# fvalka/atc-reinforcement-learning

Measured on AMD Instinct MI355X. Metric: env-steps/sec aggregate @16 aircraft/env, 64k envs, higher is better.
Workload: dtype f32

## Files before the change

### atc-reinforcement-learning_amd/csrc/atc_step.hip

```cpp
#include <hip/hip_runtime.h>
#include <atomic>
#include <chrono>
#include <sched.h>
#include <emmintrin.h>
#include <stdint.h>
#include <stdio.h>
#include <string.h>

#include "atc_device.h"

using namespace atc;

struct atc_scenario {
    float* d_blob;
    int n_words;
    int off_grid;
    int device;
    int n_cu;
    float consts[ATC_C_END];
    float ghdr[ATC_G_HDR];
    uint64_t uid;
    void* d_lds;
    LdsTab lt;
    size_t lds_tab_bytes;
// ... 641 lines not shown
            const float t2 = in_horizon ? lim.sep2 : lim.sep2_h, tf = in_horizon ? lim.sep_ft : lim.sep_ft_h;
#pragma unroll 1
            for (int d0 = H - U + 1; d0 >= 1; d0 -= U) {
                const int batch = (d0 - 1) / U;
                if (kHZ && !((batches >> batch) & 1u)) continue;
                v2f qx[U / 2], qy[U / 2], qh[U / 2];
#pragma unroll
                for (int u = 0; u < U / 2; ++u) {
                    const float* q0 = own + d0 + 2 * u;
                    qx[u] = v2f{q0[0], q0[1]};
                    qy[u] = v2f{q0[P], q0[P + 1]};
                    qh[u] = v2f{q0[2 * P], q0[2 * P + 1]};
                }
                uint64_t mk[U];
                v2f d2k[U / 2], dhk[U / 2];
#pragma unroll
                for (int u = U / 2 - 1; u >= 0; --u) {
                    const v2f dx = xs2 - qx[u], dy = ys2 - qy[u];
                    const v2f d2 = __builtin_elementwise_fma(dx, dx, dy * dy);
                    d2k[u] = d2;
                    {
                        const v2f dh = hs2 - qh[u];
                        dhk[u] = dh;
                        mk[2 * u] = __builtin_amdgcn_ballot_w64(d2[0] < t2) & __builtin_amdgcn_ballot_w64(fabsf(dh[0]) < tf);
                        mk[2 * u + 1] = __builtin_amdgcn_ballot_w64(d2[1] < t2) & __builtin_amdgcn_ballot_w64(fabsf(dh[1]) < tf);
                    }
                    if (FULL) {
#pragma unroll
                        for (int w = 1; w >= 0; --w) {
                            const int dd = d0 + 2 * u + w;
                            min_d2 = fminf(min_d2, d2[w]);
                            atomicMin(reinterpret_cast<unsigned int*>(own - k + 3 * P + ((k + dd) & (W - 1))), __float_as_uint(d2[w]));
                        }
                    }
                }
                uint64_t any = mk[0];
#pragma unroll
                for (int j = 1; j < U; ++j) any |= mk[j];
                if (ATC_RARE(any != 0ull)) {
                    if (kHZ && !in_horizon) {
                        flagged |= 1u << batch;
                        any = 0ull;
#pragma unroll
                        for (int j = 0; j < U; ++j) {
                            mk[j] = __builtin_amdgcn_ballot_w64(d2k[j / 2][j % 2] < sep2) & __builtin_amdgcn_ballot_w64(fabsf(dhk[j / 2][j % 2]) < sep_ft);
                            any |= mk[j];
                        }
                    }
                    hit |= any;
#pragma unroll
                    for (int j = 0; j < U; ++j) {
                        const int dd = d0 + j;
                        const uint64_t t = mk[j];
                        if (W == 64) {
                            hit |= (t << dd) | (t >> (64 - dd));
                        } else {
                            const uint32_t lo = (uint32_t)t, hi = (uint32_t)(t >> 32);
                            hit |= (uint64_t)((lo << dd) | (lo >> (32 - dd))) | ((uint64_t)((hi << dd) | (hi >> (32 - dd))) << 32);
                        }
                    }
                }
            }
            if ((hit >> lane) & 1ull) margin = -1.0f;
            if (FULL) {
                __builtin_amdgcn_fence(__ATOMIC_RELEASE, "wavefront");
                __builtin_amdgcn_wave_barrier();
                __builtin_amdgcn_fence(__ATOMIC_ACQUIRE, "wavefront");
                min_d2 = fminf(min_d2, own[3 * P]);
            }
            __builtin_amdgcn_wave_barrier();
        }
        if (kHZ && !in_horizon) {
            const uint64_t odd = __builtin_amdgcn_ballot_w64(a.v > kVMaxFix) | __builtin_amdgcn_ballot_w64(!(fabsf(hf) < kScanHMax));
            scan_skip = (odd != 0ull) ? 0 : kHorizon;
            scan_mask = flagged;
        }
    }
    ATC_STAMP_B(2);
    Obs ob;
    float shaping = 0.0f;
    const ObsConst oc = QGET(oc);
    constexpr bool kPrefetch = (W == 1 || (ONE && W == 16)) && kResolveAfterScan && !LDSG;
    constexpr bool kObsFirst = kPrefetch || W == 1;
    MvaPre pre;
    if (kPrefetch) pre = mva_prefetch(grid, QGET(g.gh), m.cell);
    if (kObsFirst) {
        const WideWords wo = LAT ? ww : wide_words<ONE>(m.plain, a.phi, wide_named, zk, i);
        const float phi_f = phi_real(wo.counts), phi_o = __int_as_float(wo.obs_bits);
        ob = get_state(oc, a.x, a.y, x32, y32, hf, phi_f, phi_o, v_real(a.v), hf);
        if (p.mode & ATC_M_REWARD_SHAPING) shaping = shaping_total(shaping_core(oc, ob.d_faf, ob.phi_rel_faf, ob.o[9], hf, ob.on_gp));
    }
    ATC_STAMP_TOP(so.trace, 5);
    if (LDSG) {
        float hgt = 0.0f;
        uint32_t walk;
        bool band;
        pi = lds_resolve(ltab, *lt, m.lc, x32, y32, &hgt, &walk, &band);
        if (ATC_RARE(__builtin_amdgcn_ballot_w64(walk != 0u) != 0ull)) {
            if (walk != 0u) pi = lds_walk(*lt, walk, x32, y32, &hgt);
            asm volatile("" : "+v"(pi), "+v"(hgt));
        }
        if (ATC_RARE(__builtin_amdgcn_ballot_w64(band) != 0ull)) {
            const GridHdr gh = QGET(g.gh);
            const MvaCell c = mva_cell_load(grid, gh, x32, y32);
            pi = mva_resolve<kWalkBatch>(K, grid, gh, c, x32, y32, &hgt);
            asm volatile("" : "+v"(pi), "+v"(hgt));
        }
        mva = hgt;
    } else if (kResolveAfterScan) {
        float hgt = 0.0f;
        pi = mva_resolve<kWalkBatch>(K, grid, QGET(g.gh), m.cell, x32, y32, &hgt, kPrefetch ? &pre : nullptr);
        mva = hgt;
        fl |= noise_areas(K, grid, qs.n_noise, m.cell, x32, y32, a.h);
    }
    ATC_STAMP_END(so.trace, 1);
    const bool conflict = margin < 0.0f;
    const bool timeout = es.t > qs.timestep_limit;
    const uint64_t in_tri = LDSG ? __builtin_amdgcn_ballot_w64(lds_corridor_candidate(m.lc))
                          : grid ? __builtin_amdgcn_ballot_w64(corridor_candidate(m.cell))
                                 : (__builtin_amdgcn_ballot_w64(x32 >= qs.tri_bbox.x) & __builtin_amdgcn_ballot_w64(x32 <= qs.tri_bbox.z) &
                                    __builtin_amdgcn_ballot_w64(y32 >= qs.tri_bbox.y) & __builtin_amdgcn_ballot_w64(y32 <= qs.tri_bbox.w));
    const double mva_d = (double)mva;
    const bool quiet = m.plain &&
                       (__builtin_amdgcn_ballot_w64(pi < 0) | __builtin_amdgcn_ballot_w64(a.h < mva_d) | __builtin_amdgcn_ballot_w64(margin < 0.0f) |
                        __builtin_amdgcn_ballot_w64(es.t > qs.timestep_limit) | __builtin_amdgcn_ballot_w64(fl > 0xffffu) | in_tri) == 0ull;
    if (ATC_RARE(!quiet)) {
        {
            const bool below = pi >= 0 && a.h < mva_d;
            r = pi < 0 ? -50.0f : (below ? -200.0f : r);
            fl |= pi < 0 ? (uint32_t)ATC_F_OUTSIDE : (below ? (uint32_t)ATC_F_BELOW_MVA : 0u);
        }
        {
            r = conflict ? qs.conflict_reward : r;
            fl |= conflict ? (uint32_t)ATC_F_CONFLICT : 0u;
        }
        if (inside_corridor(K, qs.tri_bbox, x32, y32, hf, (double)(LAT ? ww.counts : heading_counts<ONE>(m.plain, a.phi, wide_named, zk, i)))) {
            int bonus = (qs.timestep_limit - es.t) * 5;
            bonus = bonus < 0 ? 0 : bonus;
            r = (float)(10000 + bonus);
            fl |= ATC_F_WON;
        }
        {
            r = timeout ? -200.0f : r;
            fl |= timeout ? (uint32_t)ATC_F_TIMEOUT : 0u;
        }
    }
    ATC_STAMP_B(3);
    ATC_STAMP_END(so.trace, 2);
    const QNorm qn = QGET(n);
    float o[ATC_OBS_DIM];
    float zraw[ATC_OBS_DIM];
    {
        if (kObsFirst) {
            ob.o[5] = alt_above(a.h, mva);
        } else {
            const WideWords wo = LAT ? ww : wide_words<ONE>(m.plain, a.phi, wide_named, zk, i);
            const float phi_f = phi_real(wo.counts), phi_o = __int_as_float(wo.obs_bits);
            ob = get_state(oc, a.x, a.y, x32, y32, hf, phi_f, phi_o, v_real(a.v), alt_above(a.h, mva));
            if (p.mode & ATC_M_REWARD_SHAPING) shaping = shaping_total(shaping_core(oc, ob.d_faf, ob.phi_rel_faf, ob.o[9], hf, ob.on_gp));
        }
        if (p.mode & ATC_M_REWARD_SHAPING) r += shaping;
        if (ATC_RARE(!quiet && __builtin_amdgcn_ballot_w64((fl >> 16) != 0u) != 0ull)) {
            const int n_noise = qs.n_noise;
            for (int q = 0; q < n_noise; ++q)
                if ((fl >> (16 + q)) & 1u) r -= (K + (int)K[ATC_H_OFF_POLY] + ((int)K[ATC_H_N_MVA] + q) * ATC_P_WORDS)[ATC_P_PENALTY];
            fl &= 0xffffu;
        }
        if (FULL) {
#pragma unroll
            for (int c = 0; c < ATC_OBS_DIM; ++c) zraw[c] = active ? ob.o[c] : 0.0f;
            if (so.raw_obs && d.lane_valid) store_obs(at<float>(so.raw_obs, times40(i)), zraw);
        }
#pragma unroll
        for (int c = 0; c < ATC_OBS_DIM; ++c) o[c] = fmaf(ob.o[c], qn.a[c], qn.b[c]);
    }
    if (ATC_RARE(!m.plain && __builtin_amdgcn_ballot_w64(!active) != 0ull)) {
#pragma unroll
        for (int c = 0; c < ATC_OBS_DIM; ++c) o[c] = active ? o[c] : 0.0f;
        r = active ? r : 0.0f;
        acts = active ? acts : 0;
        fl = active ? fl : (d.lane_valid ? (uint32_t)ATC_F_INACTIVE : 0u);
        if (!active) min_d2 = 1e30f;
    }

    ATC_STAMP_B(4);
    ATC_STAMP_END(so.trace, 3);
    const float env_r = group_sum<W>(r);
    const int env_acts = m.repeated ? 0 : group_sum_i<W>(acts);
    bool done = false, env_won = false;
    if (ATC_RARE(!quiet)) {
        const uint64_t won = group_ballot<W>((fl & ATC_F_WON) != 0, lane);
        const uint64_t term = group_ballot<W>(
            (fl & (ATC_F_BELOW_MVA | ATC_F_OUTSIDE | ATC_F_CONFLICT | ATC_F_TIMEOUT)) != 0, lane);
        const bool keep_active = (p.mode & ATC_M_KEEP_ACTIVE) != 0;
        if (!keep_active) es.amask &= ~won;
        env_won = keep_active ? won != 0 : es.amask == 0;
        done = d.env_valid && (term != 0 || env_won);
        if (kHZ && (p.mode & ATC_M_AUTO_RESET) && __builtin_amdgcn_ballot_w64(done) != 0ull) scan_skip = 0;
    }
    es.total_reward += env_r;
    es.n_actions += env_acts;

    if (FULL && ONE && W == 1 && so.packet && d.lane_valid) {
        const uint32_t tag = p.reserved0;
        const float w[27] = {o[0], o[1], o[2], o[3], o[4], o[5], o[6], o[7], o[8], o[9], zraw[0], zraw[1], zraw[2], zraw[3],
                             zraw[4], zraw[5], zraw[6], zraw[7], zraw[8], zraw[9], env_r,
                             __uint_as_float((fl & 0xffffu) | (done ? 0x10000u : 0u)), __int_as_float(es.t),
                             __int_as_float(es.n_actions), __int_as_float(a.x), __int_as_float(a.y), 0.0f};
        uint4* pk = at<uint4>(so.packet, (uint32_t)e * (ATC_PKT_CHUNKS * 16u));
#pragma unroll
        for (int c = 0; c < ATC_PKT_CHUNKS; ++c)
            store16_system(pk + c, __float_as_uint(w[3 * c]), __float_as_uint(w[3 * c + 1]), __float_as_uint(w[3 * c + 2]), tag);
    }
    if (FULL && so.min_sep) {
        const float m2 = (W > 1) ? group_min<W>(min_d2) : 1e30f;
        if (d.env_valid && k == 0) *at<float>(so.min_sep, (uint32_t)e * 4u) = (m2 >= 1e30f) ? 1e30f : sqrtf(m2);
    }

    if (ATC_RARE(done && (p.mode & ATC_M_AUTO_RESET))) {
        __builtin_amdgcn_fence(__ATOMIC_ACQUIRE, "wavefront");
        int32_t* stats = ONE ? stp : kernarg_reread<int32_t*>(offsetof(StepArgs, st) + offsetof(atc_state_t, stats), zk);
        int4* sr = at<int4>(stats, (uint32_t)e * (ATC_STAT_WORDS * 4u));
        const int4 s0 = sr[0];
        const int episode = s0.x;
        if (d.env_valid && k == 0) {
            const uint32_t win_bits = (((uint32_t)s0.w << 1) | (env_won ? 1u : 0u)) & 0x3ffu;
            sr[0] = make_int4(episode + 1, es.t, __float_as_int(es.total_reward), (int)win_bits);
            *at<int>(stats, (uint32_t)e * (ATC_STAT_WORDS * 4u) + ATC_STAT_EP_ACTIONS * 4u) = es.n_actions;
        }
        __builtin_amdgcn_fence(__ATOMIC_RELEASE, "wavefront");
        if (d.lane_valid) {
            if (FULL && so.term_obs) store_obs(at<float>(so.term_obs, times40(i)), o);
            a = spawn(K, qs.off_spawn, p, e, k + zk, episode, o);
        }
        es.total_reward = 0.0f;
        es.n_actions = 0;
        es.t = 0;
        es.amask = (N >= 64) ? ~0ull : ((1ull << N) - 1ull);
    }

    ATC_STAMP_B(5);
    ATC_STAMP_END(so.trace, 4);
    if (!ONE && !LAT) {
        int zn;
        asm volatile("s_mov_b32 %0, 0" : "=s"(zn));
        qr_next = kernarg_reread<QRates>(offsetof(StepArgs, q) + offsetof(StepDerived, r), zn);
    }
    if (ATC_RARE(act_next != nullptr)) asm volatile("" : "+v"(a_next.a), "+v"(a_next.b), "+v"(a_next.c));
    if (ATC_USUAL(d.wave_full)) {
        const uint32_t ln = threadIdx.x & 63u, wv = threadIdx.x >> 6;
        float* tb = obs_stage + __umul24(wv, 64u * ATC_OBS_DIM);
        float2* tb2 = reinterpret_cast<float2*>(tb) + __umul24(ln, ATC_OBS_DIM / 2);
#pragma unroll
        for (int c = 0; c < ATC_OBS_DIM / 2; ++c) tb2[c] = make_float2(o[2 * c], o[2 * c + 1]);
        __builtin_amdgcn_fence(__ATOMIC_RELEASE, "wavefront");
        __builtin_amdgcn_wave_barrier();
        __builtin_amdgcn_fence(__ATOMIC_ACQUIRE, "wavefront");
        const uint32_t wave_off = (d.slot0 + (uint32_t)__builtin_amdgcn_readfirstlane((int)(threadIdx.x & ~63u))) * 40u;
        const float4* src = reinterpret_cast<const float4*>(tb);
#pragma unroll
        for (int j = 0; j < 3; ++j) {
            const uint32_t idx = (uint32_t)j * 64u + ln;
            if (idx < 64u * ATC_OBS_DIM / 4u) {
                const float4 v = src[idx];
                float* d4 = at<float>(so.obs, wave_off + idx * 16u);
                typedef float v4f __attribute__((ext_vector_type(4)));
                __builtin_nontemporal_store(v4f{v.x, v.y, v.z, v.w}, reinterpret_cast<v4f*>(d4));
            }
        }
        __builtin_amdgcn_wave_barrier();
    } else if (d.lane_valid) {
        store_obs(at<float>(so.obs, times40(i)), o);
    }
    ATC_STAMP_END(so.trace, 5);
    if (d.lane_valid) {
        stream_store(at<uint16_t>(so.flags, i * 2u), (uint16_t)fl);
        if (FULL && so.ac_reward) *at<float>(so.ac_reward, i * 4u) = r;
    }
    if (d.env_valid && k == 0) {
        *at<float>(so.reward, (uint32_t)e * 4u) = env_r;
        *at<uint8_t>(so.done, (uint32_t)e) = done ? 1 : 0;
    }
    return quiet;
}

__device__ __forceinline__ void store_lane_state(const atc_state_t& st, const LaneIds& d, const LaneState& ls, bool la_live) {
    if (d.lane_valid) {
        *at<int4>(st.ac, d.i * 16u) = make_int4(ls.a.x, ls.a.y, ls.a.phi, (int)ls.a.v);
        *at<double>(st.alt, d.i * 8u) = ls.a.h;
    }
    if (__builtin_amdgcn_ballot_w64(ls.la_changed) != 0ull && d.lane_valid && la_live)
        *at<int4>(st.last_act, d.i * 16u) = make_int4((int)ls.la_v, ls.la_p, __double2loint(ls.la_h), __double2hiint(ls.la_h));
}
template <int W>
__device__ __forceinline__ void store_env_state(const atc_state_t& st, const LaneIds& d, const EnvState& es, uint32_t hi0) {
    if (d.env_valid && d.k == 0) {
        *at<int4>(st.env, (uint32_t)d.e * (ATC_ENV_WORDS * 4u)) =
            make_int4(es.t, es.n_actions, __float_as_int(es.total_reward), (int)(uint32_t)(es.amask & 0xffffffffu));
        if (W == 64 && (uint32_t)(es.amask >> 32) != hi0)
            *at<uint32_t>(st.stats, (uint32_t)d.e * (ATC_STAT_WORDS * 4u) + ATC_STAT_MASK_HI * 4u) = (uint32_t)(es.amask >> 32);
    }
}

#define ATC_LAT_WAVES 2
template <int W, bool FULL, bool ONE, bool ALLV, bool LAT = false, bool LDSG = false>
__global__ void __launch_bounds__(kBlock, (LDSG ? 1 : LAT ? ATC_LAT_WAVES : ONE ? ATC_MIN_WAVES : ((FULL || W <= 8 || W >= 32) ? ATC_MIN_WAVES_LOOP - 1 : ATC_MIN_WAVES_LOOP)))
k_step(const float* __restrict__ blob, int off_grid, int B, int N, int T, int hold, atc_state_t st,
       const float* __restrict__ actions, atc_out_t out, atc_params_t p, StepDerived q_arg, InlineAction ia, LdsTab lt_arg) {
    static_assert(!LAT || (!ONE && !FULL), "LAT is an instantiation of the fast multi-step kernels");
    static_assert(!LDSG || (LAT && W == 1 && ALLV), "LDSG is an instantiation of the latency-bound one-aircraft kernel");
    StepDerived q_vec;
    if (LAT) q_vec = to_vector_registers(q_arg);
    const StepDerived& q = LAT ? q_vec : q_arg;
    extern __shared__ __attribute__((aligned(16))) float smem[];
    float4* pos = reinterpret_cast<float4*>(smem);
    float* obs_stage = smem + (W >= 32 ? 2 * kBlock * 4 : 0);
    const float* __restrict__ K = blob;
    const float* __restrict__ grid = off_grid ? blob + off_grid : nullptr;
#if ATC_TRACE
    const int tid = threadIdx.x, lane = tid & 63;
    unsigned long long* trace = reinterpret_cast<unsigned long long*>(
        ((unsigned long long)p.reserved0) | ((unsigned long long)__float_as_uint(p.reserved1) << 32));
    const unsigned long long t_launch = __builtin_amdgcn_s_memtime();
#endif
    const uint32_t BN = (uint32_t)B * (uint32_t)N;
#define ATC_KARG_PREFETCH(W, ONE) ((ONE) && (W) <= 16)
    int karg_touch = 0;
    if (ATC_KARG_PREFETCH(W, ONE)) {
#if __HIP_DEVICE_COMPILE__
        typedef __attribute__((address_space(4))) const int* karg_ip;
        karg_ip kb = (karg_ip)__builtin_amdgcn_kernarg_segment_ptr();
#pragma unroll
        for (int ln = 1; ln < (int)((offsetof(StepArgs, lt) + 63) / 64); ++ln) karg_touch ^= kb[16 * ln];
#endif
    }
    const LaneIds d = make_ids<W, ALLV>(blockIdx.x * kBlock, B, N);

    const int4 e0 = *at<int4>(st.env, (uint32_t)d.e * (ATC_ENV_WORDS * 4u));
    const uint32_t hi0 = (W == 64) ? *at<uint32_t>(st.stats, (uint32_t)d.e * (ATC_STAT_WORDS * 4u) + ATC_STAT_MASK_HI * 4u) : 0u;
    EnvState es = {e0.x, e0.y, __int_as_float(e0.z), (uint64_t)(uint32_t)e0.w | ((uint64_t)hi0 << 32)};
    const int4 ps = *at<int4>(st.ac, d.i * 16u);
    const double h0 = *at<double>(st.alt, d.i * 8u);
    Float3 act = {0.0f, 0.0f, 0.0f};
    if (ONE && W == 1 && FULL && ia.set) {
        act = Float3{ia.v, ia.h, ia.p};
    } else if (ONE) {
        act = *at<Float3>(actions, times12(d.i));
    }
    const bool same_actions = ONE && (p.mode & ATC_M_ACTIONS_HELD) != 0;
    const bool la_live = !same_actions || e0.x == 0;
    int4 la0 = make_int4(0, 0, 0, 0);
    if (la_live) la0 = *at<int4>(st.last_act, d.i * 16u);
    LaneState ls = {{ps.x, ps.y, h0, ps.z, (uint32_t)ps.w}, (uint32_t)la0.x, __hiloint2double(la0.w, la0.z), la0.y, false};

    const int n_steps = ONE ? 1 : T;
    const float* act_t = actions;
    int left = hold;
    bool block_start = true;
    Targets tg = {0u, 0.0f, 0};
    uint64_t refused_blk = 0ull;
    bool refused_known = false;
    bool all_active = false, mask_dirty = true;
    int scan_skip = 0;
    uint32_t scan_mask = 0u;
    QRates qr_next = q.r;
    if (!ONE && !LAT) {
        int zn;
        asm volatile("s_mov_b32 %0, 0" : "=s"(zn));
        qr_next = kernarg_reread<QRates>(offsetof(StepArgs, q) + offsetof(StepDerived, r), zn);
    }
    LdsTab ltv = lt_arg;
    const char* ltab = nullptr;
    if (LDSG) {
        uint4* dst = reinterpret_cast<uint4*>(smem + (kBlock / 64) * 64 * ATC_OBS_DIM);
        const int n16 = lt_arg.n16;
        constexpr int kDepth = 28;
        for (int base = 0; base < n16; base += kDepth * kBlock) {
            uint4 v[kDepth];
#pragma unroll
            for (int u = 0; u < kDepth; ++u) {
                const int j = base + u * kBlock + (int)threadIdx.x;
                v[u] = lt_arg.src[min(j, n16 - 1)];
            }
#pragma unroll
            for (int u = 0; u < kDepth; ++u) asm volatile("" : "+v"(v[u].x), "+v"(v[u].y), "+v"(v[u].z), "+v"(v[u].w));
#pragma unroll
            for (int u = 0; u < kDepth; ++u) {
                const int j = base + u * kBlock + (int)threadIdx.x;
                if (j < n16) dst[j] = v[u];
            }
        }
        __syncthreads();
        ltab = reinterpret_cast<const char*>(dst);
        ltv.x0 = vg(lt_arg.x0); ltv.y0 = vg(lt_arg.y0); ltv.inv = vg(lt_arg.inv);
        ltv.nx = vg(lt_arg.nx); ltv.nx_last = vg(lt_arg.nx_last); ltv.ny_last = vg(lt_arg.ny_last);
        ltv.off_l1 = vg(lt_arg.off_l1); ltv.off_sub = vg(lt_arg.off_sub); ltv.off_line = vg(lt_arg.off_line); ltv.off_hts = vg(lt_arg.off_hts);
        ltv.off_resid = vg(lt_arg.off_resid);
    }
    if (!ONE) {
        asm volatile("" : "+v"(ls.a.x), "+v"(ls.a.y), "+v"(ls.a.h), "+v"(ls.a.phi), "+v"(ls.a.v));
        asm volatile("" : "+v"(ls.la_v), "+v"(ls.la_h), "+v"(ls.la_p), "+v"(es.t), "+v"(es.n_actions), "+v"(es.total_reward));
        uint32_t m_lo = (uint32_t)es.amask, m_hi = (uint32_t)(es.amask >> 32);
        asm volatile("" : "+v"(m_lo), "+v"(m_hi));
        es.amask = (uint64_t)m_lo | ((uint64_t)m_hi << 32);
    }
    for (int step = 0; step < n_steps; ++step) {
#if ATC_TRACE
        unsigned long long* trow = trace ? trace + ((size_t)(blockIdx.x * (kBlock / 64) + (tid >> 6)) * n_steps + step) * 8 : nullptr;
        if (lane == 0 && trow) trow[0] = step ? __builtin_amdgcn_s_memtime() : t_launch;
#endif
        const size_t sBN = (size_t)step * BN, sB = (size_t)step * (uint32_t)B;
        LaneIds dl = d;
        const float* Kl = K;
        const float* gl = grid;
        atc_params_t pl = p;
        atc_out_t outl = out;
        int32_t* stats_l = st.stats;
        int zk = 0;
        if (!ONE) {
            asm volatile("s_mov_b32 %0, 0" : "=s"(zk));
            pl.mode += (uint32_t)zk;
        }
        StepOut so = {outl.obs + sBN * ATC_OBS_DIM, outl.flags + sBN, outl.reward + sB, outl.done + sB,
                      FULL && outl.raw_obs ? outl.raw_obs + sBN * ATC_OBS_DIM : nullptr,
                      FULL && outl.ac_reward ? outl.ac_reward + sBN : nullptr,
                      FULL && outl.min_sep ? outl.min_sep + sB : nullptr,
                      FULL && outl.term_obs ? outl.term_obs + sBN * ATC_OBS_DIM : nullptr,
                      FULL && outl.packet ? outl.packet + sB * (ATC_PKT_CHUNKS * 4) : nullptr
#if ATC_TRACE
                      , trow
#endif
        };
        const QRates qr = qr_next;
        const QScan qs = QGET(s);
        if (!ONE && ATC_RARE(step == 0)) act = *at<Float3>(act_t, times12(dl.i));
        if (ONE || step == 0) tg = decode_targets(qr, act);
        if (ONE && !la_live) {
            ls.la_v = tg.v;
            ls.la_h = altitude_target(qr, tg.ah);
            ls.la_p = tg.p;
        }
        const bool repeated = ONE ? (same_actions && __builtin_amdgcn_ballot_w64(la_live) == 0ull)
                                  : (!block_start && __builtin_amdgcn_ballot_w64(es.t == 0) == 0ull);
        if (!ONE && ATC_RARE(mask_dirty)) {
            all_active = (__builtin_amdgcn_ballot_w64(!(dl.lane_valid && ((dl.k < 32 ? ((uint32_t)es.amask >> dl.k) : ((uint32_t)(es.amask >> 32) >> (dl.k - 32))) & 1u))) |
                          __builtin_amdgcn_ballot_w64(max(ls.a.phi, ls.la_p) == INT32_MAX) | __builtin_amdgcn_ballot_w64(min(ls.a.phi, ls.la_p) == INT32_MIN)) == 0ull;
            mask_dirty = false;
        }
        ATC_STAMP_TOP(trow, 1);
        const Mid m = step_part_a<ONE, LAT, LDSG>(gl, qr, QGET(k), QGET(g), dl, tg.v, altitude_target(qr, tg.ah), tg.p, act.c, ls, es, repeated, !ONE && all_active,
                                             st.phi_wide, zk, refused_blk, refused_known ATC_TRACE_PASS(trow), ltab, &ltv);
        refused_known = true;
        ATC_STAMP(1);
        Float3 nxt = act;
        const float* act_next = nullptr;
        block_start = false;
        if (!ONE && ATC_RARE(--left == 0)) {
            left = kernarg_reread<int>(offsetof(StepArgs, hold), zk);
            block_start = true;
            refused_known = false;
            act_t += (size_t)BN * 3;
            if (step + 1 < n_steps) act_next = act_t;
        }
        const bool quiet = step_part_b<W, FULL, ONE, LAT, LDSG>(Kl, gl, pl, q, qs, zk, N, dl, m, ls, es, so, stats_l, st.phi_wide, pos, obs_stage, act_next, nxt, qr_next, scan_skip, scan_mask, ltab, &ltv);
        if (ATC_RARE(!quiet)) mask_dirty = true;
        if (act_next) tg = decode_targets(QGET(r), nxt);
        act = nxt;
        ATC_STAMP(6);
        ATC_STAMP_TOP(trow, 6);
        ATC_STAMP_END(trow, 6);
    }
    atc_state_t st_end = st;
    if (ONE || loop_rereads_state(W)) {
        int zk;
        asm volatile("s_mov_b32 %0, 0" : "=s"(zk));
        st_end = kernarg_reread<atc_state_t>(offsetof(StepArgs, st), zk);
    }
    store_lane_state(st_end, d, ls, la_live);
    store_env_state<W>(st_end, d, es, hi0);
    if (ATC_KARG_PREFETCH(W, ONE)) asm volatile("" ::"s"(karg_touch));
#if ATC_TRACE
    if (lane == 0 && trace) trace[((size_t)(blockIdx.x * (kBlock / 64) + (tid >> 6)) * n_steps + (n_steps - 1)) * 8 + 7] = __builtin_amdgcn_s_memtime();
#endif
}

enum { ATC_MB_CMD = 0, ATC_MB_SEQ = 3, ATC_MB_STATE = 4, ATC_MB_LAST = 5, ATC_MB_WORDS = 16 };
enum { ATC_SERVE_IDLE = 0, ATC_SERVE_RUNNING = 1, ATC_SERVE_LEFT_LEASE = 2, ATC_SERVE_LEFT_QUIT = 3 };
#define ATC_SERVE_QUIT 0xffffffffu
__device__ __forceinline__ uint32_t mb_load(const uint32_t* w) {
    return __hip_atomic_load(w, __ATOMIC_RELAXED, __HIP_MEMORY_SCOPE_SYSTEM);
}
__global__ void __launch_bounds__(64, 1)
k_serve(const float* __restrict__ blob, int off_grid, atc_state_t st, atc_out_t out, atc_params_t p, StepDerived q_arg,
        uint32_t* mailbox, uint32_t last, unsigned long long lease_ticks) {
    const StepDerived q = to_vector_registers(q_arg);
    extern __shared__ __attribute__((aligned(16))) float smem[];
    const float* __restrict__ K = blob;
    const float* __restrict__ grid = off_grid ? blob + off_grid : nullptr;
    const LaneIds d = make_ids<1, false>(0u, 1, 1);
    const int4 e0 = *at<int4>(st.env, 0u);
    EnvState es = {e0.x, e0.y, __int_as_float(e0.z), (uint64_t)(uint32_t)e0.w};
    const int4 ps = *at<int4>(st.ac, 0u);
    const double h0 = *at<double>(st.alt, 0u);
    const int4 la0 = *at<int4>(st.last_act, 0u);
    LaneState ls = {{ps.x, ps.y, h0, ps.z, (uint32_t)ps.w}, (uint32_t)la0.x, __hiloint2double(la0.w, la0.z), la0.y, false};
    const StepOut so = {out.obs, out.flags, out.reward, out.done, out.raw_obs, out.ac_reward, out.min_sep, out.term_obs, out.packet
#if ATC_TRACE
                        , nullptr
#endif
    };
    if (threadIdx.x == 0) __hip_atomic_store(mailbox + ATC_MB_STATE, (uint32_t)ATC_SERVE_RUNNING, __ATOMIC_RELEASE, __HIP_MEMORY_SCOPE_SYSTEM);
    unsigned long long t_cmd = __builtin_amdgcn_s_memrealtime();
    uint32_t left_as = ATC_SERVE_LEFT_LEASE;
    for (;;) {
        const uint32_t seq = (uint32_t)__builtin_amdgcn_readfirstlane((int)__hip_atomic_load(mailbox + ATC_MB_SEQ, __ATOMIC_ACQUIRE, __HIP_MEMORY_SCOPE_SYSTEM));
        if (seq == ATC_SERVE_QUIT) {
            left_as = ATC_SERVE_LEFT_QUIT;
            break;
        }
        if (seq != last + 1u) {
            if (__builtin_amdgcn_s_memrealtime() - t_cmd > lease_ticks) break;
            continue;
        }
        const Float3 act = {__uint_as_float(mb_load(mailbox + ATC_MB_CMD)), __uint_as_float(mb_load(mailbox + ATC_MB_CMD + 1)),
                            __uint_as_float(mb_load(mailbox + ATC_MB_CMD + 2))};
        last = seq;
        atc_params_t pl = p;
        pl.reserved0 = seq;
        const Targets tg = decode_targets(q.r, act);
        uint64_t refused = 0ull;
        const Mid m = step_part_a<true, true>(grid, q.r, q.k, q.g, d, tg.v, altitude_target(q.r, tg.ah), tg.p, act.c, ls, es, false, false,
                                               st.phi_wide, 0, refused, false ATC_TRACE_PASS(nullptr));
        Float3 nxt = act;
        QRates qn = q.r;
        int scan_skip = 0;
        uint32_t scan_mask = 0u;
        step_part_b<1, true, true, true>(K, grid, pl, q, q.s, 0, 1, d, m, ls, es, so, st.stats, st.phi_wide, nullptr, smem, nullptr, nxt, qn,
                                          scan_skip, scan_mask);
        t_cmd = __builtin_amdgcn_s_memrealtime();
    }
    store_lane_state(st, d, ls, true);
    store_env_state<1>(st, d, es, 0u);
    __threadfence_system();
    if (threadIdx.x == 0) {
        __hip_atomic_store(mailbox + ATC_MB_LAST, last, __ATOMIC_RELAXED, __HIP_MEMORY_SCOPE_SYSTEM);
        __hip_atomic_store(mailbox + ATC_MB_STATE, left_as, __ATOMIC_RELEASE, __HIP_MEMORY_SCOPE_SYSTEM);
    }
}

#include "atc_aux_kernels.inc"

static int grid_for(const atc_scenario* s, long long threads) {
    long long blocks = (threads + kBlock - 1) / kBlock;
    const long long cap = (long long)s->n_cu * ATC_GRID_CAP;
    if (blocks > cap) blocks = cap;
    if (blocks < 1) blocks = 1;
    return (int)blocks;
}
static size_t lds_bytes(const atc_scenario*, bool pair_scan, bool step_kernel = false) {
    size_t w = 0;
    if (step_kernel) w += (size_t)(kBlock / 64) * 64 * ATC_OBS_DIM;
    if (pair_scan) w += (size_t)2 * kBlock * 4;
    return w * sizeof(float);
}

static thread_local uint64_t t_launches[ATC_LAUNCH_SLOTS] = {0};

template <int W, bool FULL, bool ONE, bool ALLV, bool LAT = false, bool LDSG = false>
static int launch_step2(const atc_scenario* s, int B, int N, int T, int hold, const atc_state_t* st, const float* actions,
                        const atc_out_t* out, const atc_params_t* p, hipStream_t stream) {
    const size_t lds = lds_bytes(s, W >= 32, true) + (LDSG ? s->lds_tab_bytes : 0);
    if (lds > 48 * 1024) {
        static thread_local int raised_for = -1;
        if (raised_for != s->device) {
            HIP_TRY(hipFuncSetAttribute(reinterpret_cast<const void*>(&k_step<W, FULL, ONE, ALLV, LAT, LDSG>),
                                        hipFuncAttributeMaxDynamicSharedMemorySize, s->max_lds));
            raised_for = s->device;
        }
    }
    const long long slots = (long long)B * W;
    const int grid = (int)((slots + kBlock - 1) / kBlock);
    LdsTab lt = s->lt;
    if (!LDSG) lt.src = nullptr;
    hipLaunchKernelGGL((k_step<W, FULL, ONE, ALLV, LAT, LDSG>), dim3(grid), dim3(kBlock), lds, stream, s->d_blob, s->off_grid, B, N, T, hold, *st, actions, *out, *p, derive(*p, s, scan_horizon<W, FULL, ONE>()), inline_action(), lt);
    HIP_TRY(hipGetLastError());
    constexpr int form = LDSG ? ATC_LF_LDSG : LAT ? ATC_LF_LAT : FULL ? (ONE ? ATC_LF_FULL_ONE : ATC_LF_FULL_MULTI)
                         : ONE ? (ALLV ? ATC_LF_ALLV_ONE : ATC_LF_GEN_ONE) : (ALLV ? ATC_LF_ALLV_MULTI : ATC_LF_GEN_MULTI);
    ++t_launches[__builtin_ctz(W) * ATC_LF_FORMS + form];
    return ATC_OK;
}
template <int W>
static int launch_step(const atc_scenario* s, int B, int N, int T, int hold, const atc_state_t* st, const float* actions,
                       const atc_out_t* out, const atc_params_t* p, hipStream_t stream) {
    const bool full = out->raw_obs || out->ac_reward || out->min_sep || out->term_obs || out->packet;
    const bool allv = !full && N == W && ((long long)B * W) % kBlock == 0;
    if (T > 1) {
        if (full) return launch_step2<W, true, false, false>(s, B, N, T, hold, st, actions, out, p, stream);
        const bool lat = allv && ((long long)B * W + 63) / 64 <= (long long)ATC_LAT_WAVES * 4 * s->n_cu;
        if constexpr (W == 1) {
            if (lat && s->lt.src && (long long)B <= (long long)kBlock * s->n_cu && s->off_grid &&
                lds_bytes(s, false, true) + s->lds_tab_bytes <= (size_t)s->max_lds)
                return launch_step2<1, false, false, true, true, true>(s, B, N, T, hold, st, actions, out, p, stream);
        }
        if (lat) return launch_step2<W, false, false, true, true>(s, B, N, T, hold, st, actions, out, p, stream);
        return allv ? launch_step2<W, false, false, true>(s, B, N, T, hold, st, actions, out, p, stream)
                    : launch_step2<W, false, false, false>(s, B, N, T, hold, st, actions, out, p, stream);
    }
    if (full) return launch_step2<W, true, true, false>(s, B, N, 1, 1, st, actions, out, p, stream);
    return allv ? launch_step2<W, false, true, true>(s, B, N, 1, 1, st, actions, out, p, stream)
                : launch_step2<W, false, true, false>(s, B, N, 1, 1, st, actions, out, p, stream);
}

static int check_env_args(const atc_scenario_t* s, int B, int N, const atc_state_t* st, const atc_params_t* p) {
    if (!s || !st || !p) return fail_arg("null pointer");
    if (B < 1 || N < 1 || N > ATC_MAX_AIRCRAFT) return fail_arg("need B >= 1, 1 <= N <= 64");
    if (!st->ac || !st->alt || !st->last_act || !st->env || !st->stats || !st->phi_wide) return fail_arg("atc_state_t has a null field");
    if ((unsigned long long)B * N * ATC_OBS_DIM * 4ull >= (1ull << 32) || (unsigned long long)B * 64ull >= (1ull << 32))
        return fail_arg("B*N too large for one launch (B*N*40 bytes must stay below 4 GiB): split the batch");
    return ATC_OK;
}

static int step_common(const atc_scenario_t* s, int B, int N, int T, int hold, const atc_state_t* st, const float* actions,
                       const atc_out_t* out, const atc_params_t* p, void* stream) {
    if (!actions || !out) return fail_arg("null pointer");
    if (const int rc = check_env_args(s, B, N, st, p)) return rc;
    if (T < 1 || hold < 1) return fail_arg("need T >= 1 and hold >= 1");
    if (T % hold != 0) return fail_arg("T must be a multiple of hold (actions holds T / hold blocks)");
    if (!out->obs || !out->reward || !out->done || !out->flags) return fail_arg("obs/reward/done/flags are required");
    if (out->packet && (N != 1 || T != 1)) return fail_arg("atc_out_t.packet is for single steps of single-aircraft envs");
    if (!(p->dt > 0.0)) return fail_arg("dt must be > 0");
    if (!(0.1423 * p->dt * (double)s->consts[ATC_C_POS_SCALE] < 1073741824.0) || !((double)kAMax * p->dt < 255.9))
        return fail_arg("dt too large for the fixed-point state formats (see include/atc_step.h)");
    hipStream_t q = (hipStream_t)stream;
    if (N == 1) return launch_step<1>(s, B, N, T, hold, st, actions, out, p, q);
    if (N == 2) return launch_step<2>(s, B, N, T, hold, st, actions, out, p, q);
    if (N <= 4) return launch_step<4>(s, B, N, T, hold, st, actions, out, p, q);
    if (N <= 8) return launch_step<8>(s, B, N, T, hold, st, actions, out, p, q);
    if (N <= 16) return launch_step<16>(s, B, N, T, hold, st, actions, out, p, q);
    if (N <= 32) return launch_step<32>(s, B, N, T, hold, st, actions, out, p, q);
    return launch_step<64>(s, B, N, T, hold, st, actions, out, p, q);
}

#include "atc_abi.inc"
```

Baseline: 3.402 billion.

## Process two block tiles per workgroup in the 16-aircraft single-step kernel

```diff
diff --git a/atc-reinforcement-learning_amd/csrc/atc_step.hip b/atc-reinforcement-learning_amd/csrc/atc_step.hip
--- a/atc-reinforcement-learning_amd/csrc/atc_step.hip
+++ b/atc-reinforcement-learning_amd/csrc/atc_step.hip
@@ -967,6 +967,120 @@
     }
 }
 
+struct StepTile {
+    LaneIds d;
+    LaneState ls;
+    EnvState es;
+    Float3 act;
+    bool la_live;
+#if ATC_TRACE
+    unsigned long long* trow;
+#endif
+};
+__device__ __forceinline__ void tile_load(StepTile& t, const atc_state_t& st, const float* __restrict__ actions) {
+    const int4 e0 = *at<int4>(st.env, (uint32_t)t.d.e * (ATC_ENV_WORDS * 4u));
+    const int4 ps = *at<int4>(st.ac, t.d.i * 16u);
+    const double h0 = *at<double>(st.alt, t.d.i * 8u);
+    t.act = *at<Float3>(actions, times12(t.d.i));
+    t.es = {e0.x, e0.y, __int_as_float(e0.z), (uint64_t)(uint32_t)e0.w};
+    t.ls = {{ps.x, ps.y, h0, ps.z, (uint32_t)ps.w}, 0u, 0.0, 0, false};
+}
+__device__ __forceinline__ void tile_load_last(StepTile& t, const atc_state_t& st, bool same_actions) {
+    t.la_live = !same_actions || t.es.t == 0;
+    int4 la0 = make_int4(0, 0, 0, 0);
+    if (t.la_live) la0 = *at<int4>(st.last_act, t.d.i * 16u);
+    t.ls.la_v = (uint32_t)la0.x;
+    t.ls.la_h = __hiloint2double(la0.w, la0.z);
+    t.ls.la_p = la0.y;
+}
+__device__ __forceinline__ Mid tile_part_a(StepTile& t, const float* __restrict__ grid, const StepDerived& q, double* wide_named,
+                                           bool same_actions, const LdsTab* ltv) {
+    const Targets tg = decode_targets(q.r, t.act);
+    if (!t.la_live) {
+        t.ls.la_v = tg.v;
+        t.ls.la_h = altitude_target(q.r, tg.ah);
+        t.ls.la_p = tg.p;
+    }
+    const bool repeated = same_actions && __builtin_amdgcn_ballot_w64(t.la_live) == 0ull;
+    uint64_t refused = 0ull;
+    return step_part_a<true, false>(grid, q.r, q.k, q.g, t.d, tg.v, altitude_target(q.r, tg.ah), tg.p, t.act.c, t.ls, t.es, repeated,
+                                    false, wide_named, 0, refused, false ATC_TRACE_PASS(t.trow), nullptr, ltv);
+}
+template <int W>
+__device__ __forceinline__ void tile_part_b(StepTile& t, const Mid& m, const float* __restrict__ K, const float* __restrict__ grid,
+                                            const atc_params_t& p, const StepDerived& q, int N, const atc_state_t& st, const atc_out_t& out,
+                                            float* obs_stage, const LdsTab* ltv) {
+    const StepOut so = {out.obs, out.flags, out.reward, out.done, nullptr, nullptr, nullptr, nullptr, nullptr
+#if ATC_TRACE
+                        , t.trow
+#endif
+    };
+    Float3 nxt = t.act;
+    QRates qr_next = q.r;
+    int scan_skip = 0;
+    uint32_t scan_mask = 0u;
+    step_part_b<W, false, true, false>(K, grid, p, q, q.s, 0, N, t.d, m, t.ls, t.es, so, st.stats, st.phi_wide,
+                                       reinterpret_cast<float4*>(obs_stage), obs_stage, nullptr, nxt, qr_next, scan_skip, scan_mask,
+                                       nullptr, ltv);
+    int zk;
+    asm volatile("s_mov_b32 %0, 0" : "=s"(zk));
+    const atc_state_t st_end = kernarg_reread<atc_state_t>(offsetof(StepArgs, st), zk);
+    store_lane_state(st_end, t.d, t.ls, t.la_live);
+    store_env_state<W>(st_end, t.d, t.es, 0u);
+#if ATC_TRACE
+    if ((threadIdx.x & 63) == 0 && t.trow) t.trow[7] = __builtin_amdgcn_s_memtime();
+#endif
+}
+template <int W>
+__device__ __forceinline__ void step_tiles(const float* __restrict__ K, const float* __restrict__ grid, float* obs_stage, int B, int N,
+                                           const atc_state_t& st, const float* __restrict__ actions, const atc_out_t& out,
+                                           const atc_params_t& p, const StepDerived& q, const LdsTab& lt_arg) {
+    static_assert(W == 16, "two tiles per wavefront: the all-valid single step of 16-aircraft envs");
+#if ATC_TRACE
+    unsigned long long* trace = reinterpret_cast<unsigned long long*>(
+        ((unsigned long long)p.reserved0) | ((unsigned long long)__float_as_uint(p.reserved1) << 32));
+    const unsigned long long t_launch = __builtin_amdgcn_s_memtime();
+#endif
+    int karg_touch = 0;
+#if __HIP_DEVICE_COMPILE__
+    typedef __attribute__((address_space(4))) const int* karg_ip;
+    karg_ip kb = (karg_ip)__builtin_amdgcn_kernarg_segment_ptr();
+#pragma unroll
+    for (int ln = 1; ln < (int)((offsetof(StepArgs, lt) + 63) / 64); ++ln) karg_touch ^= kb[16 * ln];
+#endif
+    const uint32_t BN = (uint32_t)B * (uint32_t)N;
+    const bool two = gridDim.x * (uint32_t)kBlock < BN;
+    const uint32_t slot_a = blockIdx.x * (two ? 2u * kBlock : (uint32_t)kBlock);
+    const bool has_b = two && slot_a + kBlock < BN;
+    const bool same_actions = (p.mode & ATC_M_ACTIONS_HELD) != 0;
+    const LdsTab ltv = lt_arg;
+    StepTile ta, tb;
+    ta.d = make_ids<W, true>(slot_a, B, N);
+    tb.d = make_ids<W, true>(slot_a + kBlock, B, N);
+#if ATC_TRACE
+    ta.trow = trace ? trace + (size_t)(slot_a / 64u + (threadIdx.x >> 6)) * 8 : nullptr;
+    tb.trow = trace ? trace + (size_t)((slot_a + kBlock) / 64u + (threadIdx.x >> 6)) * 8 : nullptr;
+    if ((threadIdx.x & 63) == 0 && ta.trow) ta.trow[0] = t_launch;
+    if (has_b && (threadIdx.x & 63) == 0 && tb.trow) tb.trow[0] = t_launch;
+#endif
+    if (has_b) {
+        tile_load(ta, st, actions);
+        tile_load(tb, st, actions);
+        tile_load_last(ta, st, same_actions);
+        tile_load_last(tb, st, same_actions);
+        const Mid ma = tile_part_a(ta, grid, q, st.phi_wide, same_actions, &ltv);
+        const Mid mb = tile_part_a(tb, grid, q, st.phi_wide, same_actions, &ltv);
+        tile_part_b<W>(ta, ma, K, grid, p, q, N, st, out, obs_stage, &ltv);
+        tile_part_b<W>(tb, mb, K, grid, p, q, N, st, out, obs_stage, &ltv);
+    } else {
+        tile_load(ta, st, actions);
+        tile_load_last(ta, st, same_actions);
+        const Mid ma = tile_part_a(ta, grid, q, st.phi_wide, same_actions, &ltv);
+        tile_part_b<W>(ta, ma, K, grid, p, q, N, st, out, obs_stage, &ltv);
+    }
+    asm volatile("" ::"s"(karg_touch));
+}
+
 #define ATC_LAT_WAVES 2
 template <int W, bool FULL, bool ONE, bool ALLV, bool LAT = false, bool LDSG = false>
 __global__ void __launch_bounds__(kBlock, (LDSG ? 1 : LAT ? ATC_LAT_WAVES : ONE ? ATC_MIN_WAVES : ((FULL || W <= 8 || W >= 32) ? ATC_MIN_WAVES_LOOP - 1 : ATC_MIN_WAVES_LOOP)))
@@ -982,6 +1096,10 @@
     float* obs_stage = smem + (W >= 32 ? 2 * kBlock * 4 : 0);
     const float* __restrict__ K = blob;
     const float* __restrict__ grid = off_grid ? blob + off_grid : nullptr;
+    if constexpr (ONE && ALLV && W == 16) {
+        step_tiles<W>(K, grid, obs_stage, B, N, st, actions, out, p, q, lt_arg);
+        return;
+    }
 #if ATC_TRACE
     const int tid = threadIdx.x, lane = tid & 63;
     unsigned long long* trace = reinterpret_cast<unsigned long long*>(
@@ -1231,6 +1349,17 @@
 
 static thread_local uint64_t t_launches[ATC_LAUNCH_SLOTS] = {0};
 
+#ifndef ATC_TWO_TILE_WAVES
+#define ATC_TWO_TILE_WAVES 4
+#endif
+static bool step_two_tiles(const atc_scenario* s, long long slots) {
+    if (const char* f = getenv("ATC_STEP_TILES")) {
+        if (!strcmp(f, "1")) return false;
+        if (!strcmp(f, "2")) return true;
+    }
+    return slots / 64 > (long long)ATC_TWO_TILE_WAVES * 4 * s->n_cu;
+}
+
 template <int W, bool FULL, bool ONE, bool ALLV, bool LAT = false, bool LDSG = false>
 static int launch_step2(const atc_scenario* s, int B, int N, int T, int hold, const atc_state_t* st, const float* actions,
                         const atc_out_t* out, const atc_params_t* p, hipStream_t stream) {
@@ -1244,7 +1373,10 @@
         }
     }
     const long long slots = (long long)B * W;
-    const int grid = (int)((slots + kBlock - 1) / kBlock);
+    int grid = (int)((slots + kBlock - 1) / kBlock);
+    if constexpr (ONE && ALLV && W == 16) {
+        if (step_two_tiles(s, slots)) grid = (int)((slots + 2 * kBlock - 1) / (2 * kBlock));
+    }
     LdsTab lt = s->lt;
     if (!LDSG) lt.src = nullptr;
     hipLaunchKernelGGL((k_step<W, FULL, ONE, ALLV, LAT, LDSG>), dim3(grid), dim3(kBlock), lds, stream, s->d_blob, s->off_grid, B, N, T, hold, *st, actions, *out, *p, derive(*p, s, scan_horizon<W, FULL, ONE>()), inline_action(), lt);
```

After: 3.143 billion. -7.6%, worse.
